# jasperzhong/GNNFlow

Measured on AMD Instinct MI355X. Metric: sampled_edges_per_s, higher is better.
Workload: dtype int64/f32

## Files before the change

gnnflow_amd/csrc/sample_layer.hip:

```cpp
#include "sampler_ctx.hpp"

#include <cstdlib>

#include "../../include/gnnflow_rng.h"

namespace gf {

namespace {

__global__ void sample_publish_kernel(Publish p) {
  if (threadIdx.x != 0 || blockIdx.x != 0) return;
  for (uint32_t i = 0; i < p.num_words; ++i) p.h_counts[i] = p.d_counts[i];
  p.h_counts[p.num_words] = p.d_extra ? *p.d_extra : 0;
  __threadfence_system();
  *reinterpret_cast<volatile uint64_t*>(p.h_flag) = p.seq;
}

__global__ void sample_publish_group_kernel(PublishGroup g) {
  if (threadIdx.x != 0) return;
  const Publish& p = g.p[blockIdx.x];
  for (uint32_t i = 0; i < p.num_words; ++i) p.h_counts[i] = p.d_counts[i];
  p.h_counts[p.num_words] = p.d_extra ? *p.d_extra : 0;
  __threadfence_system();
  *reinterpret_cast<volatile uint64_t*>(p.h_flag) = p.seq;
}

template <int GROUP>
__global__ __launch_bounds__(kSearchThreads) void sample_search_kernel(
    GraphView g, const int64_t* __restrict__ roots, const float* __restrict__ root_ts,
    const uint64_t* __restrict__ d_R, uint64_t R_host, uint32_t snapshot_idx,
    uint32_t num_snapshots, float window, uint64_t* __restrict__ rec_end,
    uint32_t* __restrict__ rec_cnt, uint32_t fanout, int uniform,
    uint32_t* __restrict__ wg_sum, const uint32_t* __restrict__ list,
    const uint32_t* __restrict__ seg_count, uint32_t num_segs, uint32_t seg_cap) {
  __shared__ uint32_t s_sum;
  __shared__ uint32_t seg_prefix[kMaxHubSegs + 1];
  if (wg_sum && threadIdx.x == 0) s_sum = 0;
  if (wg_sum) __syncthreads();
  uint64_t R = d_R ? *d_R : R_host;
  if (list) {
    __shared__ uint32_t wtot[kSearchThreads / 64];
    uint32_t carry = 0;
    for (uint32_t s0 = 0; s0 < num_segs; s0 += kSearchThreads) {
      const uint32_t sidx = s0 + threadIdx.x;
      const uint32_t v = sidx < num_segs ? seg_count[sidx] : 0u;
      uint32_t incl = v;
#pragma unroll
      for (int d = 1; d < 64; d <<= 1) {
        const uint32_t up = __shfl_up(incl, d, 64);
        if ((threadIdx.x & 63) >= d) incl += up;
      }
      __syncthreads();
      if ((threadIdx.x & 63) == 63) wtot[threadIdx.x >> 6] = incl;
      __syncthreads();
      uint32_t wbase = 0, tot = 0;
      for (int w = 0; w < kSearchThreads / 64; ++w) {
        if (w < (threadIdx.x >> 6)) wbase += wtot[w];
        tot += wtot[w];
      }
      if (sidx < num_segs) seg_prefix[sidx] = carry + wbase + incl - v;
      carry += tot;
    }
    if (threadIdx.x == 0) seg_prefix[num_segs] = carry;
    __syncthreads();
    R = seg_prefix[num_segs];
  }
  constexpr int kGroupsPerBlock = kSearchThreads / GROUP;
  const int lane = threadIdx.x % GROUP;
  const int group_in_wave = (threadIdx.x % 64) / GROUP;
  const uint64_t group = static_cast<uint64_t>(blockIdx.x) * kGroupsPerBlock + threadIdx.x / GROUP;
  const uint64_t num_groups = static_cast<uint64_t>(gridDim.x) * kGroupsPerBlock;
  for (uint64_t i = group; i < R; i += num_groups) {
    uint64_t r = i;
    if (list) {
      uint32_t lo_s = 0, hi_s = num_segs;
      while (hi_s - lo_s > 1) {
        const uint32_t mid = (lo_s + hi_s) >> 1;
        if (seg_prefix[mid] <= i) lo_s = mid; else hi_s = mid;
      }
      r = list[static_cast<uint64_t>(lo_s) * seg_cap + (i - seg_prefix[lo_s])];
    }
    const int64_t nid = roots[r];
    const float t = root_ts[r];
    float start, end;
    time_window(t, snapshot_idx, num_snapshots, window, &start, &end);
    uint64_t end_off = 0;
    uint32_t n_cand = 0;
    if (nid >= 0 && static_cast<uint64_t>(nid) < g.table_len) {
      const NodeEntry e = g.table[nid];
      if (e.size > 0) {
        uint32_t lo, hi;
        window_bounds<GROUP>(g, e, start, end, lane, group_in_wave, &lo, &hi);
        n_cand = hi > lo ? hi - lo : 0;
        end_off = e.start + hi;
      }
    }
    if (lane == 0) {
      rec_end[r] = end_off;
      rec_cnt[r] = n_cand;
      if (wg_sum) atomicAdd(&s_sum, valid_slots(n_cand, fanout, uniform));
    }
  }
  if (wg_sum) {
    __syncthreads();
    if (threadIdx.x == 0) wg_sum[blockIdx.x] = s_sum;
  }
}

constexpr uint32_t kLaneDeg = 16;

__global__ __launch_bounds__(kSearchThreads) void sample_search_lanes_kernel(
    GraphView g, const int64_t* __restrict__ roots, const float* __restrict__ root_ts,
    const uint64_t* __restrict__ d_R, uint64_t R_host, uint32_t snapshot_idx,
    uint32_t num_snapshots, float window, uint64_t* __restrict__ rec_end,
    uint32_t* __restrict__ rec_cnt, uint32_t* __restrict__ hub_list,
    uint32_t* __restrict__ seg_count, uint32_t seg_cap) {
  __shared__ uint32_t s_seg_n;
  if (threadIdx.x == 0) s_seg_n = 0;
  __syncthreads();
  uint32_t* seg = hub_list + static_cast<uint64_t>(blockIdx.x) * seg_cap;
  const uint64_t R = d_R ? *d_R : R_host;
  const int lane = threadIdx.x & 63;
  const uint64_t wave = (static_cast<uint64_t>(blockIdx.x) * kSearchThreads + threadIdx.x) >> 6;
  const uint64_t num_waves = (static_cast<uint64_t>(gridDim.x) * kSearchThreads) >> 6;
  const uint64_t chunks = (R + 63) / 64;
  for (uint64_t chunk = wave; chunk < chunks; chunk += num_waves) {
    const uint64_t r = chunk * 64 + lane;
    const bool in = r < R;
    int64_t nid = -1;
    float start = 0.f, end = 0.f;
    if (in) {
      nid = roots[r];
      time_window(root_ts[r], snapshot_idx, num_snapshots, window, &start, &end);
    }
    NodeEntry e;
    e.start = 0;
    e.size = 0;
    if (in && nid >= 0 && static_cast<uint64_t>(nid) < g.table_len) e = g.table[nid];
    const bool whole = g.nonneg_ts > 0 && start <= 0.0f && e.size > 0 &&
                       end > __uint_as_float(e.last_ts_bits);
    const bool big = e.size > kLaneDeg && !whole;
    if (in && whole) {
      rec_end[r] = e.start + e.size;
      rec_cnt[r] = e.size;
    } else if (in && !big) {
      uint32_t hi = 0, lo = 0;
      if (e.size > 0) {
        const float* ts = g.ts_pool + e.start;
        float v[kLaneDeg];
        if ((e.start & 3u) == 0) {
          const float4* t4 = reinterpret_cast<const float4*>(ts);
#pragma unroll
          for (uint32_t q = 0; q < kLaneDeg / 4; ++q) {
            const float4 x = 4 * q < e.size ? t4[q] : make_float4(0.f, 0.f, 0.f, 0.f);
            v[4 * q] = x.x; v[4 * q + 1] = x.y; v[4 * q + 2] = x.z; v[4 * q + 3] = x.w;
          }
        } else {
#pragma unroll
          for (uint32_t i = 0; i < kLaneDeg; ++i) v[i] = i < e.size ? ts[i] : 0.f;
// ... 181 lines not shown
    pub.h_counts[pub.num_words] = 0;
  }
  const uint64_t stride = static_cast<uint64_t>(gridDim.x) * blockDim.x;
  const uint64_t first = static_cast<uint64_t>(blockIdx.x) * blockDim.x + threadIdx.x;
  constexpr int K = 4;
  for (uint64_t t0 = first; t0 < total; t0 += K * stride) {
    uint64_t t[K], r[K], end[K];
    uint32_t j[K], n[K], bs[K];
    float rts[K];
    bool in[K];
#pragma unroll
    for (int k = 0; k < K; ++k) {
      t[k] = t0 + static_cast<uint64_t>(k) * stride;
      in[k] = t[k] < total;
      r[k] = in[k] ? t[k] / fanout : 0;
      j[k] = static_cast<uint32_t>(t[k] - r[k] * fanout);
    }
#pragma unroll
    for (int k = 0; k < K; ++k) {
      n[k] = in[k] ? rec_cnt[r[k]] : 0u;
      end[k] = in[k] ? rec_end[r[k]] : 0;
      bs[k] = in[k] ? base[r[k]] : 0u;
      rts[k] = in[k] ? root_ts[r[k]] : 0.f;
      if (in[k] && t[k] < R) {
        all_nodes[t[k]] = roots[t[k]];
        all_ts[t[k]] = root_ts[t[k]];
      }
    }
    EdgePair nb[K];
    bool ok[K];
#pragma unroll
    for (int k = 0; k < K; ++k) {
      ok[k] = in[k] && j[k] < valid_slots(n[k], fanout, uniform);
      if (ok[k]) {
        const uint32_t pick = uniform ? gf_philox4x32_10_first(seed, t[k], call) % n[k] : j[k];
        nb[k] = g.nbr_pool[end[k] - 1 - pick];
      }
    }
#pragma unroll
    for (int k = 0; k < K; ++k) {
      if (!ok[k]) continue;
      const float ets = nb[k].ts;
      const uint64_t o = static_cast<uint64_t>(bs[k]) + j[k];
      all_nodes[R + o] = nb[k].dst;
      all_ts[R + o] = prop_time ? rts[k] : ets;
      dt[o] = rts[k] - ets;
      eids[o] = nb[k].eid;
      row[o] = static_cast<int64_t>(r[k]);
      col[o] = static_cast<int64_t>(R + o);
    }
  }
}

__global__ __launch_bounds__(kEmitThreads) void sample_emit_prefix_kernel(
    GraphView g, const int64_t* __restrict__ roots, const float* __restrict__ root_ts,
    const uint64_t* d_R, uint64_t R_host, uint32_t fanout, int uniform, int prop_time,
    uint64_t seed, uint64_t call, const uint64_t* __restrict__ rec_end,
    const uint32_t* __restrict__ rec_cnt, const uint32_t* __restrict__ wg_sum,
    uint32_t roots_per_search_wg, int64_t* __restrict__ all_nodes, float* __restrict__ all_ts,
    float* __restrict__ dt, int64_t* __restrict__ eids, int64_t* __restrict__ row,
    int64_t* __restrict__ col, uint64_t* out_R, uint64_t* out_S, uint64_t* next_R, Publish pub) {
  __shared__ uint32_t red[kEmitThreads / 64];
  __shared__ uint32_t lbase[kEmitThreads];
  __shared__ uint32_t wave_tot[kEmitThreads / 64];
  const uint64_t R = d_R ? *d_R : R_host;
  const uint64_t total = R * fanout;
  const uint64_t t0 = static_cast<uint64_t>(blockIdx.x) * kEmitThreads;
  if (t0 >= total) return;
  const int tid = threadIdx.x, lane = tid & 63, wave = tid >> 6;
  const uint64_t t_last = min(t0 + kEmitThreads - 1, total - 1);
  const uint32_t r_first = static_cast<uint32_t>(t0 / fanout);
  const uint32_t r_last = static_cast<uint32_t>(t_last / fanout);
  const uint32_t nroots = r_last - r_first + 1;
  const uint32_t b_first = r_first / roots_per_search_wg;
  uint32_t part = 0;
  for (uint32_t b = tid; b < b_first; b += kEmitThreads) part += wg_sum[b];
  for (uint32_t r = b_first * roots_per_search_wg + tid; r < r_first; r += kEmitThreads)
    part += valid_slots(rec_cnt[r], fanout, uniform);
  for (int d = 32; d > 0; d >>= 1) part += __shfl_down(part, d, 64);
  if (lane == 0) red[wave] = part;
  const uint32_t mine = tid < static_cast<int>(nroots)
                            ? valid_slots(rec_cnt[r_first + tid], fanout, uniform) : 0u;
  uint32_t incl = mine;
#pragma unroll
  for (int d = 1; d < 64; d <<= 1) {
    uint32_t up = __shfl_up(incl, d, 64);
    if (lane >= d) incl += up;
  }
  if (lane == 63) wave_tot[wave] = incl;
  __syncthreads();
  uint32_t base = 0;
#pragma unroll
  for (int w = 0; w < kEmitThreads / 64; ++w) base += red[w];
  uint32_t wbase = 0;
  for (int w = 0; w < wave; ++w) wbase += wave_tot[w];
  lbase[tid] = base + wbase + incl - mine;
  __syncthreads();
  const uint64_t t = t0 + tid;
  if (t < total) {
    if (t < R) {
      all_nodes[t] = roots[t];
      all_ts[t] = root_ts[t];
    }
    const uint32_t r = static_cast<uint32_t>(t / fanout);
    const uint32_t j = static_cast<uint32_t>(t - static_cast<uint64_t>(r) * fanout);
    const uint32_t n = rec_cnt[r];
    if (j < valid_slots(n, fanout, uniform)) {
      const uint32_t pick = uniform ? gf_philox4x32_10_first(seed, t, call) % n : j;
      const uint64_t e = rec_end[r] - 1 - pick;
      const EdgePair nb = g.nbr_pool[e];
      const float ets = nb.ts;
      const float rts = root_ts[r];
      const uint64_t o = static_cast<uint64_t>(lbase[r - r_first]) + j;
      all_nodes[R + o] = nb.dst;
      all_ts[R + o] = prop_time ? rts : ets;
      dt[o] = rts - ets;
      eids[o] = nb.eid;
      row[o] = static_cast<int64_t>(r);
      col[o] = static_cast<int64_t>(R + o);
    }
  }
  if (t_last == total - 1 && tid == static_cast<int>(nroots) - 1) {
    const uint64_t S = static_cast<uint64_t>(lbase[tid]) + mine;
    *out_R = R;
    *out_S = S;
    if (next_R) *next_R = R + S;
    for (uint32_t i = 0; i < pub.num_words; ++i) pub.h_counts[i] = pub.d_counts[i];
    if (pub.num_words) pub.h_counts[pub.num_words] = 0;
  }
}

template <typename... Args>
void launch_search(int width, unsigned grid, hipStream_t stream, Args... args) {
  switch (width) {
    case 2: sample_search_kernel<2><<<dim3(grid), dim3(kSearchThreads), 0, stream>>>(args...); break;
    case 4: sample_search_kernel<4><<<dim3(grid), dim3(kSearchThreads), 0, stream>>>(args...); break;
    case 8: sample_search_kernel<8><<<dim3(grid), dim3(kSearchThreads), 0, stream>>>(args...); break;
    default: sample_search_kernel<16><<<dim3(grid), dim3(kSearchThreads), 0, stream>>>(args...); break;
  }
}

}

int group_width_from_env(const char* name, int fallback) {
  const char* v = std::getenv(name);
  const int g = v ? std::atoi(v) : fallback;
  return (g == 2 || g == 4 || g == 8 || g == 16) ? g : fallback;
}

void launch_scan(const uint32_t* rec_cnt, uint32_t* base, uint32_t* tile_scratch,
                 const uint64_t* d_R, uint64_t R_host, size_t Rb, uint32_t F, int uniform,
                 uint64_t* out_R, uint64_t* out_S, uint64_t* next_R, hipStream_t stream) {
  if (Rb <= 65536) {
    sample_scan_kernel<<<dim3(1), dim3(kScanThreads), 0, stream>>>(
        rec_cnt, base, d_R, R_host, F, uniform, out_R, out_S, next_R);
    return;
  }
  const size_t tiles = (Rb + kScanTile - 1) / kScanTile;
  uint32_t* tile_sum = tile_scratch;
  uint32_t* tile_base = tile_scratch + tiles;
  const unsigned grid = static_cast<unsigned>(std::min<size_t>(tiles, 2048));
  sample_tile_sum_kernel<<<dim3(grid), dim3(kScanThreads), 0, stream>>>(
      rec_cnt, d_R, R_host, F, uniform, tile_sum);
  sample_tile_scan_kernel<<<dim3(1), dim3(kScanThreads), 0, stream>>>(
      tile_sum, tile_base, d_R, R_host, out_R, out_S, next_R);
  sample_tile_apply_kernel<<<dim3(grid), dim3(kScanThreads), 0, stream>>>(
      rec_cnt, tile_base, d_R, R_host, F, uniform, base);
}

void launch_publish(const Publish& p, hipStream_t stream) {
  sample_publish_kernel<<<dim3(1), dim3(64), 0, stream>>>(p);
}
void launch_publish_group(const PublishGroup& g, int m, hipStream_t stream) {
  sample_publish_group_kernel<<<dim3(static_cast<unsigned>(m)), dim3(64), 0, stream>>>(g);
}

void Sampler::enqueue_layer(const int64_t* d_roots, const float* d_ts, size_t Rb,
                            const uint64_t* d_R, uint64_t R_host, uint32_t layer,
                            uint32_t snapshot, const BlockPtrs& out, uint64_t* d_counts_slot,
                            uint64_t* next_R, hipStream_t stream, const Publish& pub) {
  const uint32_t F = fanouts_[layer];
  const int uniform = policy_ == GF_SAMPLING_POLICY_UNIFORM;
  GF_REQUIRE(static_cast<uint64_t>(Rb) * F < 0xFFFFFFFFull,
             "sampler: more than 2^32-1 slots in one layer");
  char* w = ws_.as<char>();
  uint64_t* rec_end = reinterpret_cast<uint64_t*>(w); w += align_up(ws_roots_ * 8, 16);
  uint32_t* rec_cnt = reinterpret_cast<uint32_t*>(w); w += align_up(ws_roots_ * 4, 16);
  uint32_t* base = reinterpret_cast<uint32_t*>(w);    w += align_up(ws_roots_ * 4, 16);
  uint32_t* wg_sum = reinterpret_cast<uint32_t*>(w);
  const GraphView gv = view_for(graph_, Rb);
  const uint64_t call = calls_++;
  const bool small = Rb <= kSmallRoots;
  const unsigned roots_per_wg = kSearchThreads / search_group_;
  {
    ProfileScope ps(kProfSearch, stream);
    const unsigned grid = small ? static_cast<unsigned>((Rb + roots_per_wg - 1) / roots_per_wg)
                                : capped_grid(Rb, roots_per_wg, 256 * 8);
    if (hybrid_search_ && Rb >= kLaneSearchRoots) {
      const unsigned lgrid = capped_grid(Rb, kSearchThreads, kMaxHubSegs);
      const uint64_t chunks_per_wg = ((Rb + 63) / 64 + (lgrid * 4ull) - 1) / (lgrid * 4ull);
      const uint32_t seg_cap = static_cast<uint32_t>(chunks_per_wg * 4 * 64);
      const size_t hub_bytes = static_cast<size_t>(seg_cap) * lgrid * sizeof(uint32_t);
      if (hub_bytes > hub_buf_.bytes()) {
        DeviceBuffer fresh;
        fresh.reserve(hub_bytes, 0, stream);
        std::swap(hub_buf_, fresh);
        retired_.retire(std::move(fresh), stream);
      }
      uint32_t* hub_list_ = hub_buf_.as<uint32_t>();
      uint32_t* seg_count = wg_sum;
      sample_search_lanes_kernel<<<dim3(lgrid), dim3(kSearchThreads), 0, stream>>>(
          gv, d_roots, d_ts, d_R, R_host, snapshot, num_snapshots_, window_, rec_end, rec_cnt,
          hub_list_, seg_count, seg_cap);
      launch_search(large_group_, capped_grid(Rb / 4, kSearchThreads / large_group_, 256 * 8),
                    stream, gv, d_roots, d_ts, nullptr, 0, snapshot, num_snapshots_, window_,
                    rec_end, rec_cnt, F, uniform, nullptr, hub_list_, seg_count, lgrid, seg_cap);
    } else if (small) {
      launch_search(search_group_, grid, stream, gv, d_roots, d_ts, d_R, R_host, snapshot,
                    num_snapshots_, window_, rec_end, rec_cnt, F, uniform, wg_sum, nullptr,
                    nullptr, 0, 0);
    } else {
      launch_search(large_group_, capped_grid(Rb, kSearchThreads / large_group_, 256 * 8), stream,
                    gv, d_roots, d_ts, d_R, R_host, snapshot, num_snapshots_, window_, rec_end,
                    rec_cnt, F, uniform, nullptr, nullptr, nullptr, 0, 0);
    }
    GF_HIP(hipGetLastError());
  }
  if (small) {
    ProfileScope ps(kProfEmit, stream);
    const unsigned grid = static_cast<unsigned>(
        (static_cast<uint64_t>(Rb) * F + kEmitThreads - 1) / kEmitThreads);
    sample_emit_prefix_kernel<<<dim3(grid), dim3(kEmitThreads), 0, stream>>>(
        gv, d_roots, d_ts, d_R, R_host, F, uniform, prop_time_ ? 1 : 0, seed_, call, rec_end,
        rec_cnt, wg_sum, roots_per_wg, out.all_nodes, out.all_ts, out.dt, out.eids, out.row,
        out.col, d_counts_slot, d_counts_slot + 1, next_R, pub);
    GF_HIP(hipGetLastError());
    return;
  }
  {
    ProfileScope ps(kProfScan, stream);
    launch_scan(rec_cnt, base, wg_sum, d_R, R_host, Rb, F, uniform, d_counts_slot,
                d_counts_slot + 1, next_R, stream);
    GF_HIP(hipGetLastError());
  }
  {
    ProfileScope ps(kProfEmit, stream);
    unsigned grid = capped_grid(static_cast<uint64_t>(Rb) * F, kEmitThreads, 256 * 16);
    sample_emit_kernel<<<dim3(grid), dim3(kEmitThreads), 0, stream>>>(
        gv, d_roots, d_ts, d_R, R_host, F, uniform, prop_time_ ? 1 : 0, seed_, call, rec_end,
        rec_cnt, base, out.all_nodes, out.all_ts, out.dt, out.eids, out.row, out.col, pub);
    GF_HIP(hipGetLastError());
  }
}

__global__ void philox_debug_kernel(const uint64_t* __restrict__ in, size_t n,
                                    uint32_t* __restrict__ out) {
  const size_t i = static_cast<size_t>(blockIdx.x) * blockDim.x + threadIdx.x;
  if (i < n) out[i] = gf_philox4x32_10_first(in[3 * i], in[3 * i + 1], in[3 * i + 2]);
}
void philox_on_device(const uint64_t* d_in, size_t n, uint32_t* d_out, hipStream_t stream) {
  if (n == 0) return;
  philox_debug_kernel<<<dim3(static_cast<unsigned>((n + 255) / 256)), dim3(256), 0, stream>>>(
      d_in, n, d_out);
  GF_HIP(hipGetLastError());
}

}
```

gnnflow_amd/csrc/sampler.hip:

```cpp
#include "sampler_ctx.hpp"
#include "partition.hpp"

#include <sched.h>

#include <atomic>
#include <chrono>
#include <cmath>
#include <cstdlib>
#include <cstring>

namespace gf {

Sampler::Sampler(EdgeStore* graph, const uint32_t* fanouts, size_t num_layers, int policy,
                 uint32_t num_snapshots, float window, bool prop_time, uint64_t seed)
    : graph_(graph),
      fanouts_(fanouts, fanouts + num_layers),
      policy_(policy),
      num_snapshots_(num_snapshots),
      window_(window),
      prop_time_(prop_time),
      seed_(seed) {
  GF_REQUIRE(graph != nullptr, "sampler: null graph");
  GF_REQUIRE(num_layers > 0, "sampler: fanouts must not be empty");
  for (uint32_t f : fanouts_) GF_REQUIRE(f > 0, "sampler: fanout must be positive");
// ... 13 lines not shown
  std::memset(h_counts_.data(), 0, kMaxInFlight * rec_words_ * sizeof(uint64_t));
  h_layer_counts_.reserve(2 * sizeof(uint64_t));
}

Sampler::~Sampler() {
  for (InFlight& f : ring_) {
    if (f.done) {
      (void)hipEventSynchronize(f.done);
      (void)hipEventDestroy(f.done);
    }
  }
  if (own_stream_) {
    (void)hipStreamSynchronize(own_stream_);
    (void)hipStreamDestroy(own_stream_);
  }
}

size_t Sampler::root_bound(size_t R, size_t layer) const {
  size_t b = R;
  for (size_t l = 0; l < layer; ++l) b += b * fanouts_[l];
  return b;
}

size_t Sampler::layer_output_bytes(size_t Rb, size_t layer) const {
  const size_t F = fanouts_[layer], Sb = Rb * F;
  return align_up((Rb + Sb) * 8, 16) + align_up((Rb + Sb) * 4, 16) + align_up(Sb * 4, 16) +
         3 * align_up(Sb * 8, 16);
}

Sampler::BlockPtrs Sampler::carve(char* p, size_t Rb, uint32_t F) const {
  const size_t Sb = Rb * F;
  BlockPtrs b;
  b.all_nodes = reinterpret_cast<int64_t*>(p); p += align_up((Rb + Sb) * 8, 16);
  b.eids = reinterpret_cast<int64_t*>(p);      p += align_up(Sb * 8, 16);
  b.row = reinterpret_cast<int64_t*>(p);       p += align_up(Sb * 8, 16);
  b.col = reinterpret_cast<int64_t*>(p);       p += align_up(Sb * 8, 16);
  b.all_ts = reinterpret_cast<float*>(p);      p += align_up((Rb + Sb) * 4, 16);
  b.dt = reinterpret_cast<float*>(p);
  return b;
}

size_t Sampler::output_bytes(size_t R) const {
  size_t total = 0;
  for (size_t l = 0; l < fanouts_.size(); ++l)
    total += num_snapshots_ * layer_output_bytes(root_bound(R, l), l);
  return total;
}

void Sampler::reserve_workspace(size_t Rb, size_t num_blocks, hipStream_t stream) {
  if (Rb <= ws_roots_ && num_blocks <= ws_blocks_) return;
  ws_roots_ = std::max(ws_roots_, Rb);
  ws_blocks_ = std::max(ws_blocks_, num_blocks);
  size_t bytes = align_up(ws_roots_ * 8, 16) + 3 * align_up(ws_roots_ * 4, 16) +
                 ws_blocks_ * 2 * sizeof(uint64_t) + 64;
  retired_.collect();
  DeviceBuffer fresh;
  fresh.reserve(bytes, 0, stream);
  GF_HIP(hipMemsetAsync(fresh.data(), 0, align_up(ws_roots_ * 8, 16), stream));
  std::swap(ws_, fresh);
  retired_.retire(std::move(fresh), stream);
}

void Sampler::sample_begin(const int64_t* d_roots, const float* d_ts, size_t R, void* d_out,
                           size_t out_bytes, hipStream_t stream) {
  const size_t L = fanouts_.size(), NS = num_snapshots_;
  InFlight* slot;
  {
    std::lock_guard<std::mutex> lk(ring_mu_);
    GF_REQUIRE(ring_count_ < kMaxInFlight, "sample_begin: too many samples in flight on this sampler");
    if (ring_count_ > 0) {
      const InFlight& newest = ring_[(ring_head_ + ring_count_ - 1) % kMaxInFlight];
      GF_REQUIRE(newest.roots == 0 || R == 0 || newest.stream == stream,
                 "sample_begin: samples in flight on one sampler must share a stream");
    }
    slot = &ring_[(ring_head_ + ring_count_) % kMaxInFlight];
  }
  slot->ptrs.assign(L * NS, BlockPtrs{});
  slot->roots = R;
  slot->by_event = false;
  slot->stream = stream;
  if (R == 0) {
    calls_ += L * NS;
    std::lock_guard<std::mutex> lk(ring_mu_);
    ++ring_count_;
    return;
  }
  GF_REQUIRE(d_roots && d_ts && d_out, "sample: null device pointer");
  GF_REQUIRE(out_bytes >= output_bytes(R), "sample: output buffer too small");
  DeviceGuard dg(graph_->device());
  reserve_workspace(root_bound(R, L - 1), L * NS, stream);
  uint64_t* d_counts = reinterpret_cast<uint64_t*>(
      ws_.as<char>() + align_up(ws_roots_ * 8, 16) + 3 * align_up(ws_roots_ * 4, 16));

  std::vector<BlockPtrs>& ptrs = slot->ptrs;
  char* p = static_cast<char*>(d_out);
  for (size_t l = 0; l < L; ++l) {
    const size_t Rb = root_bound(R, l);
    for (size_t s = 0; s < NS; ++s) {
      ptrs[l * NS + s] = carve(p, Rb, fanouts_[l]);
      p += layer_output_bytes(Rb, l);
    }
  }
  slot->seq = ++publish_seq_;
  uint64_t* rec = h_counts_.as<uint64_t>() + (slot->seq % kMaxInFlight) * rec_words_;
  *reinterpret_cast<volatile uint64_t*>(rec) = 0;
  Publish pub;
  pub.d_counts = d_counts;
  pub.h_counts = rec + 1;
  pub.h_flag = rec;
  pub.seq = slot->seq;
  pub.num_words = static_cast<uint32_t>(L * NS * 2);
  slot->by_event = true;
  for (size_t l = 0; l < L; ++l) {
    const size_t Rb = root_bound(R, l);
    for (size_t s = 0; s < NS; ++s) {
      const size_t b = l * NS + s;
      uint64_t* cslot = d_counts + 2 * b;
      uint64_t* next_R = (l + 1 < L) ? cslot + 2 * NS : nullptr;
      const Publish last = (b + 1 == L * NS) ? pub : Publish{};
      if (l == 0) {
        enqueue_layer(d_roots, d_ts, Rb, nullptr, R, l, s, ptrs[b], cslot, next_R, stream, last);
      } else {
        const BlockPtrs& prev = ptrs[(l - 1) * NS + s];
        enqueue_layer(prev.all_nodes, prev.all_ts, Rb, cslot, 0, l, s, ptrs[b], cslot, next_R,
                      stream, last);
      }
    }
  }
  GF_HIP(hipEventRecord(slot->done, stream));
  std::lock_guard<std::mutex> lk(ring_mu_);
  ++ring_count_;
}

size_t Sampler::in_flight() const {
  std::lock_guard<std::mutex> lk(ring_mu_);
  return ring_count_;
}

void Sampler::sample_end(gf_block* blocks) {
  const size_t L = fanouts_.size(), NS = num_snapshots_;
  GF_REQUIRE(blocks != nullptr, "sample: null blocks array");
  InFlight* slot;
  {
    std::lock_guard<std::mutex> lk(ring_mu_);
    GF_REQUIRE(ring_count_ > 0, "sample_end: no sample in flight");
    slot = &ring_[ring_head_];
  }
  auto pop = [&] {
    std::lock_guard<std::mutex> lk(ring_mu_);
    ring_head_ = (ring_head_ + 1) % kMaxInFlight;
    --ring_count_;
  };
  if (slot->roots == 0) {
    for (size_t b = 0; b < L * NS; ++b) std::memset(&blocks[b], 0, sizeof(gf_block));
    last_overflow_ = false;
    pop();
    return;
  }
  DeviceGuard dg(graph_->device());
  const uint64_t* rec = h_counts_.as<uint64_t>() + (slot->seq % kMaxInFlight) * rec_words_;
  volatile const uint64_t* flag = rec;
  bool seen = false;
  if (slot->by_event) {
    for (uint64_t spin = 0;; ++spin) {
      const hipError_t q = hipEventQuery(slot->done);
      if (q == hipSuccess) break;
      if (q != hipErrorNotReady) { pop(); GF_HIP(q); }
      if (spin > 4096 && (spin & 63) == 0) sched_yield();
    }
    seen = true;
  }
  for (uint64_t spin = 0; !seen && spin < (1ull << 26); ++spin) {
    if (*flag == slot->seq) { seen = true; break; }
    __builtin_ia32_pause();
    if (spin > 4096 && (spin & 63) == 0) sched_yield();
  }
  if (!seen) {
    const hipError_t e = hipEventSynchronize(slot->done);
    if (e != hipSuccess) { pop(); GF_HIP(e); }
  }
  __atomic_thread_fence(__ATOMIC_ACQUIRE);
  const uint64_t* hc = rec + 1;
  for (size_t b = 0; b < L * NS; ++b) {
    gf_block& o = blocks[b];
    o.all_nodes = slot->ptrs[b].all_nodes;
    o.all_timestamps = slot->ptrs[b].all_ts;
    o.delta_timestamps = slot->ptrs[b].dt;
    o.eids = slot->ptrs[b].eids;
    o.row = slot->ptrs[b].row;
    o.col = slot->ptrs[b].col;
    o.num_dst_nodes = hc[2 * b];
    o.num_edges = hc[2 * b + 1];
    o.num_src_nodes = o.num_dst_nodes + o.num_edges;
  }
  last_overflow_ = hc[2 * L * NS] != 0;
  pop();
}

void Sampler::sample(const int64_t* d_roots, const float* d_ts, size_t R, void* d_out,
                     size_t out_bytes, gf_block* blocks, hipStream_t stream) {
  GF_REQUIRE(blocks != nullptr, "sample: null blocks array");
  sample_begin(d_roots, d_ts, R, d_out, out_bytes, stream);
  sample_end(blocks);
}

void Sampler::sample_layer(const int64_t* d_roots, const float* d_ts, size_t R, uint32_t layer,
                           uint32_t snapshot, void* d_out, size_t out_bytes, gf_block* block,
                           hipStream_t stream) {
  GF_REQUIRE(layer < fanouts_.size(), "sample_layer: layer out of range");
  GF_REQUIRE(snapshot < num_snapshots_, "sample_layer: snapshot out of range");
  GF_REQUIRE(block != nullptr, "sample_layer: null block");
  if (R == 0) {
    std::memset(block, 0, sizeof(gf_block));
    calls_++;
    return;
  }
  GF_REQUIRE(d_roots && d_ts && d_out, "sample_layer: null device pointer");
  GF_REQUIRE(out_bytes >= layer_output_bytes(R, layer), "sample_layer: output buffer too small");
  DeviceGuard dg(graph_->device());
  reserve_workspace(R, 2, stream);
  uint64_t* d_counts = reinterpret_cast<uint64_t*>(
      ws_.as<char>() + align_up(ws_roots_ * 8, 16) + 3 * align_up(ws_roots_ * 4, 16));
  BlockPtrs ptrs = carve(static_cast<char*>(d_out), R, fanouts_[layer]);
  enqueue_layer(d_roots, d_ts, R, nullptr, R, layer, snapshot, ptrs, d_counts, nullptr, stream,
                Publish{});
  GF_HIP(hipMemcpyAsync(h_layer_counts_.data(), d_counts, 2 * sizeof(uint64_t),
                        hipMemcpyDeviceToHost, stream));
  GF_HIP(hipStreamSynchronize(stream));
  const uint64_t* hc = h_layer_counts_.as<uint64_t>();
  block->all_nodes = ptrs.all_nodes;
  block->all_timestamps = ptrs.all_ts;
  block->delta_timestamps = ptrs.dt;
  block->eids = ptrs.eids;
  block->row = ptrs.row;
  block->col = ptrs.col;
  block->num_dst_nodes = hc[0];
  block->num_edges = hc[1];
  block->num_src_nodes = hc[0] + hc[1];
}

std::atomic<uint64_t> g_part_host_ns[8];
void part_host_add(int stage, uint64_t v) {
  g_part_host_ns[stage].fetch_add(v, std::memory_order_relaxed);
}

void Sampler::part_layout(size_t R0, uint32_t layer, int world_size, double slack,
                          size_t slot_roots, gf_part_layout* out, bool skip_prev) const {
  GF_REQUIRE(layer < fanouts_.size(), "part_layout: layer out of range");
  GF_REQUIRE(out != nullptr, "part_layout: null output");
  GF_REQUIRE(slack >= 0.0, "part_layout: negative slack");
  const size_t Rb = root_bound(R0, layer), F = fanouts_[layer];
  size_t stride = 0, rows = Rb;
  if (slack > 0.0) {
    const size_t Sb = root_bound(std::max<size_t>(slot_roots, 1), layer) -
                      ((skip_prev && layer > 0) ? root_bound(std::max<size_t>(slot_roots, 1), layer - 1) : 0);
    const double share = std::ceil(static_cast<double>(Sb) * slack / world_size);
    const size_t cap = std::max<size_t>(1, std::min<size_t>(Sb, static_cast<size_t>(share)));
    stride = cap + 1;
    rows = static_cast<size_t>(world_size) * stride + Rb;
    GF_REQUIRE(rows < 0xFFFFFFFFull, "part_layout: more than 2^32-1 request rows");
  }
  out->root_bound = Rb;
  out->requests = 0;
  out->replies = rows * 16;
  out->counts = out->replies + rows * F * 24;
  out->pos = out->counts + align_up(static_cast<size_t>(world_size) * 8, 16);
  out->scratch = align_up(out->pos + Rb * 4, 16);
  out->scratch_bytes = partition_scratch_bytes(Rb, world_size);
  size_t end = align_up(out->scratch + out->scratch_bytes, 256);
  out->slot_stride = stride;
  out->inbox = out->served = 0;
  if (stride) {
    const size_t slots = static_cast<size_t>(world_size) * stride;
    out->inbox = end;
    out->served = align_up(out->inbox + slots * 16, 256);
    end = align_up(out->served + slots * F * 24, 256);
  }
  out->total = end;
// ... 305 lines not shown
```

gnnflow_amd/csrc/sampler.hpp:

```cpp
#pragma once

#include <cstdint>
#include <mutex>
#include <vector>

#include "comm.hpp"
#include "common.hpp"
#include "edge_store.hpp"

namespace gf {

struct Publish;

class Sampler {
 public:
  Sampler(EdgeStore* graph, const uint32_t* fanouts, size_t num_layers, int policy,
          uint32_t num_snapshots, float window, bool prop_time, uint64_t seed);
  ~Sampler();

  size_t num_layers() const { return fanouts_.size(); }
  uint32_t fanout(size_t layer) const { return fanouts_[layer]; }
  uint32_t num_snapshots() const { return num_snapshots_; }
  int device() const { return graph_->device(); }

// ... 24 lines not shown
  void part_serve(uint32_t layer, uint32_t snapshot, void* d_ws, size_t ws_bytes,
                  bool with_own = false);
  bool last_overflow() const { return last_overflow_; }
  void part_plan_own(uint32_t layer, uint32_t snapshot, void* d_ws, size_t ws_bytes, int phases);
  void part_merge(uint32_t layer, uint32_t snapshot, void* d_ws, size_t ws_bytes);
  void part_commit();
  void part_abort();
  static constexpr int kMaxGroup = 4;
  struct GroupSample {
    Sampler* s;
    const int64_t* d_roots;
    const float* d_ts;
    size_t R;
    void* d_out;
    size_t out_bytes;
  };
  struct GroupLayout {
    size_t stride, slot_rows, own[kMaxGroup];
    size_t requests, replies, inbox, served, counts[kMaxGroup], pos[kMaxGroup], total;
    size_t first[kMaxGroup];
    size_t edge_cap, off_bytes, cslot, row_cnt, cserved, creplies;
  };
  bool group_ok(const size_t* R, int m) const;
  bool layer_reuses_roots(bool reuse_roots, size_t layer) const {
    return reuse_roots && layer > 0 && policy_ != GF_SAMPLING_POLICY_UNIFORM &&
           fanouts_[layer] == fanouts_[layer - 1];
  }
  void group_layout(const size_t* R, int m, uint32_t layer, int world, double slack,
                    size_t slot_roots, bool narrow, double edge_fill, GroupLayout* out,
                    bool reuse_roots = false) const;
  static size_t group_ws_bytes(const Sampler& a, const size_t* R, int m, int world, double slack,
                               size_t slot_roots, bool narrow, double edge_fill = 0.0,
                               bool reuse_roots = false);
  static void sample_partitioned_group(const GroupSample* gs, int m, void* d_ws, size_t ws_bytes,
                                       double slack, size_t slot_roots, Exchange* ex,
                                       hipStream_t stream, unsigned force_overflow = 0,
                                       bool narrow = false, double edge_fill = 0.0,
                                       bool reuse_roots = false);
  void sample_partitioned(const int64_t* d_roots, const float* d_ts, size_t R, void* d_out,
                          size_t out_bytes, void* d_ws, size_t ws_bytes, hipStream_t stream);
  void sample_partitioned_slotted(const int64_t* d_roots, const float* d_ts, size_t R, void* d_out,
                                  size_t out_bytes, void* d_ws, size_t ws_bytes, double slack,
                                  size_t slot_roots, Exchange& ex, bool overlap,
                                  hipStream_t stream);
  void sample_host(const int64_t* nodes, const float* ts, size_t R, gf_block* blocks);
  void sample_layer_host(const int64_t* nodes, const float* ts, size_t R, uint32_t layer,
                         uint32_t snapshot, gf_block* block);

 private:
  struct BlockPtrs {
    int64_t* all_nodes; float* all_ts; float* dt; int64_t* eids; int64_t* row; int64_t* col;
  };
  BlockPtrs carve(char* base, size_t Rb, uint32_t fanout) const;
  void enqueue_layer(const int64_t* d_roots, const float* d_ts, size_t R_bound,
                     const uint64_t* d_R, uint64_t R_host, uint32_t layer, uint32_t snapshot,
                     const BlockPtrs& out, uint64_t* d_counts_slot, uint64_t* next_R,
                     hipStream_t stream, const Publish& publish);
  void reserve_workspace(size_t R_bound_max, size_t num_blocks, hipStream_t stream);
  void to_host_blocks(const gf_block* dev, gf_block* host, size_t n, hipStream_t stream);

  EdgeStore* graph_;
  std::vector<uint32_t> fanouts_;
  int policy_;
  uint32_t num_snapshots_;
  float window_;
  bool prop_time_;
  uint64_t seed_;
  DeviceBuffer part_ticket_;
  uint32_t part_tag_ = 0;
  uint64_t calls_ = 0;
 public:
  uint64_t call_counter() const { return calls_; }
  void set_call_counter(uint64_t v) { calls_ = v; }
 private:
  int search_group_ = 16;
  int large_group_ = 4;
  bool hybrid_search_ = true;
  struct InFlight {
    size_t roots = 0;
    uint64_t seq = 0;
    hipStream_t stream = nullptr;
    hipEvent_t done = nullptr;
    bool by_event = false;
    std::vector<BlockPtrs> ptrs;
  };
  struct PartState {
    bool active = false;
    InFlight* slot = nullptr;
    const int64_t* d_roots = nullptr;
    const float* d_ts = nullptr;
    size_t R = 0, Rs = 1;
    int world = 1, rank = 0;
    double slack = 0.0;
    size_t slot_roots = 0;
    hipStream_t stream = nullptr;
  };
  uint64_t* part_counts() const;
  uint32_t* part_overflow() const;
  bool last_overflow_ = false;
  uint32_t* part_rec_cnt() const;
  uint32_t* part_root_of() const;
  bool part_own_counts(size_t root_bound) const;
  bool part_fused_merge(size_t root_bound, uint32_t fanout) const;
  void part_commit_prepare(Publish& pub);
  void part_commit_finish();
  void part_roots(uint32_t layer, uint32_t snapshot, const int64_t** roots, const float** ts,
                  const uint64_t** d_R, uint64_t* R_host) const;
  InFlight ring_[kMaxInFlight];
  size_t ring_head_ = 0, ring_count_ = 0;
  mutable std::mutex ring_mu_;
// ... 20 lines not shown
```

gnnflow_amd/csrc/sampler_ctx.hpp:

```cpp
#pragma once

#include "sampler.hpp"

#include <algorithm>

namespace gf {

constexpr int kSearchThreads = 256;
constexpr int kEmitThreads = 256;
constexpr int kScanThreads = 1024;
constexpr int kScanItems = 4;
constexpr size_t kSmallRoots = 32768;
constexpr uint32_t kGranuleSpins = 1u << 12;
constexpr size_t kLaneSearchRoots = size_t{1} << 20;
constexpr uint32_t kMaxHubSegs = 2048;
constexpr int kScanTile = 4096;
constexpr int kCompactThreads = 1024;
constexpr uint64_t kGranuleCountMask = 0x3FF;

__device__ inline void time_window(float root_ts, uint32_t snapshot_idx,
                                   uint32_t num_snapshots, float window, float* start,
                                   float* end) {
  if (num_snapshots == 1) {
    *start = (fabs(static_cast<double>(window)) < 1e-6) ? 0.0f : root_ts - window;
    *end = root_ts;
  } else {
    float k = static_cast<float>(num_snapshots - snapshot_idx - 1);
    *end = fmaf(-k, window, root_ts);
    *start = *end - window;
  }
}

template <int GROUP>
__device__ inline uint32_t group_count(bool pred, int group_in_wave) {
  unsigned long long m = __ballot(pred);
  if (GROUP == 64) return __popcll(m);
  return __popcll((m >> (group_in_wave * GROUP)) & ((1ull << GROUP) - 1ull));
}

template <int GROUP>
__device__ inline uint32_t lower_bound_group(const float* __restrict__ ts, uint32_t n,
                                             float x, int lane, int group_in_wave) {
  uint32_t lo = 0, hi = n;
  while (hi - lo > GROUP) {
    uint32_t span = hi - lo;
    uint32_t stride = (span + GROUP - 1) / GROUP;
    uint32_t p = lo + lane * stride;
    bool less = (p < hi) && (ts[p] < x);
    uint32_t c = group_count<GROUP>(less, group_in_wave);
    if (c == 0) {
      hi = lo;
    } else {
      uint32_t nlo = lo + (c - 1) * stride + 1;
      uint32_t nhi = lo + c * stride;
      hi = nhi < hi ? nhi : hi;
      lo = nlo;
    }
  }
  uint32_t p = lo + lane;
  bool less = (p < hi) && (ts[p] < x);
  return lo + group_count<GROUP>(less, group_in_wave);
}

template <int GROUP>
__device__ inline uint32_t lower_bound_fenced(const GraphView& g, uint64_t s, uint32_t n, float x,
// ... 239 lines not shown
```

Before: 762.2 million.

## Fuse next-layer neighbor search into emit kernel for small multi-layer batches

For small batches with a single snapshot, the emit kernel of layer l now also runs the time-window search for the newly produced roots of layer l+1. It writes rec_end/rec_cnt and accumulates per-workgroup slot sums into rotating fused sum buffers, so the separate search launch for the next layer is skipped. A head search kernel also zeroes the sum buffers, replacing separate memsets. This removes kernel launches and a pass over the new roots, at the cost of small 32-slot emit tiles with low occupancy per block and atomics on global sums.

```diff
diff --git a/gnnflow_amd/csrc/sample_layer.hip b/gnnflow_amd/csrc/sample_layer.hip
--- a/gnnflow_amd/csrc/sample_layer.hip
+++ b/gnnflow_amd/csrc/sample_layer.hip
@@ -23,6 +23,26 @@
   p.h_counts[p.num_words] = p.d_extra ? *p.d_extra : 0;
   __threadfence_system();
   *reinterpret_cast<volatile uint64_t*>(p.h_flag) = p.seq;
+}
+
+template <int GROUP>
+__device__ __forceinline__ void search_root(const GraphView& g, int64_t nid, float t,
+                                            uint32_t snapshot_idx, uint32_t num_snapshots,
+                                            float window, int lane, int group_in_wave,
+                                            uint64_t* end_off, uint32_t* n_cand) {
+  float start, end;
+  time_window(t, snapshot_idx, num_snapshots, window, &start, &end);
+  *end_off = 0;
+  *n_cand = 0;
+  if (nid >= 0 && static_cast<uint64_t>(nid) < g.table_len) {
+    const NodeEntry e = g.table[nid];
+    if (e.size > 0) {
+      uint32_t lo, hi;
+      window_bounds<GROUP>(g, e, start, end, lane, group_in_wave, &lo, &hi);
+      *n_cand = hi > lo ? hi - lo : 0;
+      *end_off = e.start + hi;
+    }
+  }
 }
 
 template <int GROUP>
@@ -80,21 +100,10 @@
       }
       r = list[static_cast<uint64_t>(lo_s) * seg_cap + (i - seg_prefix[lo_s])];
     }
-    const int64_t nid = roots[r];
-    const float t = root_ts[r];
-    float start, end;
-    time_window(t, snapshot_idx, num_snapshots, window, &start, &end);
-    uint64_t end_off = 0;
-    uint32_t n_cand = 0;
-    if (nid >= 0 && static_cast<uint64_t>(nid) < g.table_len) {
-      const NodeEntry e = g.table[nid];
-      if (e.size > 0) {
-        uint32_t lo, hi;
-        window_bounds<GROUP>(g, e, start, end, lane, group_in_wave, &lo, &hi);
-        n_cand = hi > lo ? hi - lo : 0;
-        end_off = e.start + hi;
-      }
-    }
+    uint64_t end_off;
+    uint32_t n_cand;
+    search_root<GROUP>(g, roots[r], root_ts[r], snapshot_idx, num_snapshots, window, lane,
+                       group_in_wave, &end_off, &n_cand);
     if (lane == 0) {
       rec_end[r] = end_off;
       rec_cnt[r] = n_cand;
@@ -105,6 +114,37 @@
     __syncthreads();
     if (threadIdx.x == 0) wg_sum[blockIdx.x] = s_sum;
   }
+}
+
+template <int GROUP>
+__global__ __launch_bounds__(kSearchThreads) void sample_search_head_kernel(
+    GraphView g, const int64_t* __restrict__ roots, const float* __restrict__ root_ts,
+    uint64_t R, uint32_t snapshot_idx, uint32_t num_snapshots, float window,
+    uint64_t* __restrict__ rec_end, uint32_t* __restrict__ rec_cnt, uint32_t fanout, int uniform,
+    uint32_t* __restrict__ wg_sum, uint32_t* __restrict__ zero, uint32_t zero_n) {
+  __shared__ uint32_t s_sum;
+  if (threadIdx.x == 0) s_sum = 0;
+  for (uint32_t i = blockIdx.x * kSearchThreads + threadIdx.x; i < zero_n;
+       i += gridDim.x * kSearchThreads)
+    zero[i] = 0;
+  __syncthreads();
+  constexpr int kGroupsPerBlock = kSearchThreads / GROUP;
+  const int lane = threadIdx.x % GROUP;
+  const int group_in_wave = (threadIdx.x % 64) / GROUP;
+  const uint64_t r = static_cast<uint64_t>(blockIdx.x) * kGroupsPerBlock + threadIdx.x / GROUP;
+  if (r < R) {
+    uint64_t end_off;
+    uint32_t n_cand;
+    search_root<GROUP>(g, roots[r], root_ts[r], snapshot_idx, num_snapshots, window, lane,
+                       group_in_wave, &end_off, &n_cand);
+    if (lane == 0) {
+      rec_end[r] = end_off;
+      rec_cnt[r] = n_cand;
+      atomicAdd(&s_sum, valid_slots(n_cand, fanout, uniform));
+    }
+  }
+  __syncthreads();
+  if (threadIdx.x == 0) wg_sum[blockIdx.x] = s_sum;
 }
 
 constexpr uint32_t kLaneDeg = 16;
@@ -392,23 +432,53 @@
   }
 }
 
-__global__ __launch_bounds__(kEmitThreads) void sample_emit_prefix_kernel(
-    GraphView g, const int64_t* __restrict__ roots, const float* __restrict__ root_ts,
-    const uint64_t* d_R, uint64_t R_host, uint32_t fanout, int uniform, int prop_time,
-    uint64_t seed, uint64_t call, const uint64_t* __restrict__ rec_end,
-    const uint32_t* __restrict__ rec_cnt, const uint32_t* __restrict__ wg_sum,
-    uint32_t roots_per_search_wg, int64_t* __restrict__ all_nodes, float* __restrict__ all_ts,
-    float* __restrict__ dt, int64_t* __restrict__ eids, int64_t* __restrict__ row,
-    int64_t* __restrict__ col, uint64_t* out_R, uint64_t* out_S, uint64_t* next_R, Publish pub) {
+struct EmitArgs {
+  GraphView g;
+  const int64_t* roots;
+  const float* root_ts;
+  const uint64_t* d_R;
+  uint64_t R_host;
+  uint32_t fanout;
+  int uniform, prop_time;
+  uint64_t seed, call;
+  const uint64_t* rec_end;
+  const uint32_t* rec_cnt;
+  const uint32_t* wg_sum;
+  uint32_t roots_per_search_wg;
+  int64_t* all_nodes; float* all_ts; float* dt; int64_t* eids; int64_t* row; int64_t* col;
+  uint64_t* out_R; uint64_t* out_S; uint64_t* next_R;
+  Publish pub;
+};
+
+struct NewRoot {
+  bool valid;
+  uint32_t o;
+  int64_t node;
+  float ts;
+};
+
+template <int TILE>
+__device__ __forceinline__ bool emit_prefix_tile(const EmitArgs& a, uint64_t* R_out, NewRoot* nr,
+                                                 uint32_t* o_first) {
+  static_assert(TILE >= 16 && TILE <= kEmitThreads, "a tile is at most one slot per thread");
   __shared__ uint32_t red[kEmitThreads / 64];
-  __shared__ uint32_t lbase[kEmitThreads];
+  __shared__ uint32_t lbase[TILE];
   __shared__ uint32_t wave_tot[kEmitThreads / 64];
-  const uint64_t R = d_R ? *d_R : R_host;
+  const int64_t* __restrict__ roots = a.roots;
+  const float* __restrict__ root_ts = a.root_ts;
+  const uint64_t* __restrict__ rec_end = a.rec_end;
+  const uint32_t* __restrict__ rec_cnt = a.rec_cnt;
+  const uint32_t* __restrict__ wg_sum = a.wg_sum;
+  const uint32_t fanout = a.fanout, roots_per_search_wg = a.roots_per_search_wg;
+  const int uniform = a.uniform;
+  const uint64_t R = a.d_R ? *a.d_R : a.R_host;
+  *R_out = R;
+  nr->valid = false;
   const uint64_t total = R * fanout;
-  const uint64_t t0 = static_cast<uint64_t>(blockIdx.x) * kEmitThreads;
-  if (t0 >= total) return;
+  const uint64_t t0 = static_cast<uint64_t>(blockIdx.x) * TILE;
+  if (t0 >= total) return false;
   const int tid = threadIdx.x, lane = tid & 63, wave = tid >> 6;
-  const uint64_t t_last = min(t0 + kEmitThreads - 1, total - 1);
+  const uint64_t t_last = min(t0 + TILE - 1, total - 1);
   const uint32_t r_first = static_cast<uint32_t>(t0 / fanout);
   const uint32_t r_last = static_cast<uint32_t>(t_last / fanout);
   const uint32_t nroots = r_last - r_first + 1;
@@ -434,40 +504,119 @@
   for (int w = 0; w < kEmitThreads / 64; ++w) base += red[w];
   uint32_t wbase = 0;
   for (int w = 0; w < wave; ++w) wbase += wave_tot[w];
-  lbase[tid] = base + wbase + incl - mine;
-  __syncthreads();
+  if (tid < TILE) lbase[tid] = base + wbase + incl - mine;
+  __syncthreads();
+  {
+    const uint32_t j0 = static_cast<uint32_t>(t0 - static_cast<uint64_t>(r_first) * fanout);
+    const uint32_t v0 = valid_slots(rec_cnt[r_first], fanout, uniform);
+    *o_first = lbase[0] + (j0 < v0 ? j0 : v0);
+  }
   const uint64_t t = t0 + tid;
-  if (t < total) {
+  if (tid < TILE && t < total) {
     if (t < R) {
-      all_nodes[t] = roots[t];
-      all_ts[t] = root_ts[t];
+      a.all_nodes[t] = roots[t];
+      a.all_ts[t] = root_ts[t];
     }
     const uint32_t r = static_cast<uint32_t>(t / fanout);
     const uint32_t j = static_cast<uint32_t>(t - static_cast<uint64_t>(r) * fanout);
     const uint32_t n = rec_cnt[r];
     if (j < valid_slots(n, fanout, uniform)) {
-      const uint32_t pick = uniform ? gf_philox4x32_10_first(seed, t, call) % n : j;
+      const uint32_t pick = uniform ? gf_philox4x32_10_first(a.seed, t, a.call) % n : j;
       const uint64_t e = rec_end[r] - 1 - pick;
-      const EdgePair nb = g.nbr_pool[e];
+      const EdgePair nb = a.g.nbr_pool[e];
       const float ets = nb.ts;
       const float rts = root_ts[r];
       const uint64_t o = static_cast<uint64_t>(lbase[r - r_first]) + j;
-      all_nodes[R + o] = nb.dst;
-      all_ts[R + o] = prop_time ? rts : ets;
-      dt[o] = rts - ets;
-      eids[o] = nb.eid;
-      row[o] = static_cast<int64_t>(r);
-      col[o] = static_cast<int64_t>(R + o);
+      a.all_nodes[R + o] = nb.dst;
+      a.all_ts[R + o] = a.prop_time ? rts : ets;
+      a.dt[o] = rts - ets;
+      a.eids[o] = nb.eid;
+      a.row[o] = static_cast<int64_t>(r);
+      a.col[o] = static_cast<int64_t>(R + o);
+      nr->valid = true;
+      nr->o = static_cast<uint32_t>(o);
+      nr->node = nb.dst;
+      nr->ts = a.prop_time ? rts : ets;
     }
   }
   if (t_last == total - 1 && tid == static_cast<int>(nroots) - 1) {
     const uint64_t S = static_cast<uint64_t>(lbase[tid]) + mine;
-    *out_R = R;
-    *out_S = S;
-    if (next_R) *next_R = R + S;
-    for (uint32_t i = 0; i < pub.num_words; ++i) pub.h_counts[i] = pub.d_counts[i];
-    if (pub.num_words) pub.h_counts[pub.num_words] = 0;
-  }
+    *a.out_R = R;
+    *a.out_S = S;
+    if (a.next_R) *a.next_R = R + S;
+    for (uint32_t i = 0; i < a.pub.num_words; ++i) a.pub.h_counts[i] = a.pub.d_counts[i];
+    if (a.pub.num_words) a.pub.h_counts[a.pub.num_words] = 0;
+  }
+  return true;
+}
+
+__global__ __launch_bounds__(kEmitThreads) void sample_emit_prefix_kernel(EmitArgs a) {
+  uint64_t R;
+  NewRoot nr;
+  uint32_t o_first;
+  emit_prefix_tile<kEmitThreads>(a, &R, &nr, &o_first);
+}
+
+struct NextSearchArgs {
+  uint32_t snapshot_idx, num_snapshots;
+  float window;
+  uint32_t fanout;
+  uint64_t* rec_end;
+  uint32_t* rec_cnt;
+  uint32_t* sum_next;
+  uint32_t* zero;
+  uint32_t zero_n;
+};
+
+template <int TILE, int GROUP>
+__global__ __launch_bounds__(kEmitThreads) void sample_emit_search_kernel(EmitArgs a,
+                                                                          NextSearchArgs s) {
+  constexpr int kAcc = TILE / 16 + 2;
+  __shared__ int64_t s_node[TILE];
+  __shared__ float s_ts[TILE];
+  __shared__ uint32_t s_acc[kAcc];
+  __shared__ uint32_t s_n;
+  const int tid = threadIdx.x;
+  for (uint32_t i = blockIdx.x * kEmitThreads + tid; i < s.zero_n; i += gridDim.x * kEmitThreads)
+    s.zero[i] = 0;
+  if (tid < kAcc) s_acc[tid] = 0;
+  if (tid == 0) s_n = 0;
+  uint64_t R;
+  NewRoot nr;
+  uint32_t o_first;
+  if (!emit_prefix_tile<TILE>(a, &R, &nr, &o_first)) return;
+  const uint32_t rpw = a.roots_per_search_wg;
+  const uint64_t t = static_cast<uint64_t>(blockIdx.x) * TILE + tid;
+  if (tid < TILE && t < R)
+    atomicAdd(&s.sum_next[t / rpw], valid_slots(a.rec_cnt[t], s.fanout, a.uniform));
+  if (nr.valid) {
+    const uint32_t p = nr.o - o_first;
+    if (p < TILE) {
+      s_node[p] = nr.node;
+      s_ts[p] = nr.ts;
+      atomicMax(&s_n, p + 1);
+    }
+  }
+  __syncthreads();
+  constexpr int kGroups = kEmitThreads / GROUP;
+  const int lane = tid % GROUP, group_in_wave = (tid % 64) / GROUP;
+  const uint32_t n_new = s_n;
+  const uint64_t first = R + o_first;
+  const uint64_t w0 = first / rpw;
+  for (uint32_t i = tid / GROUP; i < n_new; i += kGroups) {
+    uint64_t end_off;
+    uint32_t n_cand;
+    search_root<GROUP>(a.g, s_node[i], s_ts[i], s.snapshot_idx, s.num_snapshots, s.window, lane,
+                       group_in_wave, &end_off, &n_cand);
+    if (lane == 0) {
+      s.rec_end[first + i] = end_off;
+      s.rec_cnt[first + i] = n_cand;
+      const uint64_t w = (first + i) / rpw - w0;
+      if (w < kAcc) atomicAdd(&s_acc[w], valid_slots(n_cand, s.fanout, a.uniform));
+    }
+  }
+  __syncthreads();
+  if (tid < kAcc && s_acc[tid]) atomicAdd(&s.sum_next[w0 + tid], s_acc[tid]);
 }
 
 template <typename... Args>
@@ -477,6 +626,16 @@
     case 4: sample_search_kernel<4><<<dim3(grid), dim3(kSearchThreads), 0, stream>>>(args...); break;
     case 8: sample_search_kernel<8><<<dim3(grid), dim3(kSearchThreads), 0, stream>>>(args...); break;
     default: sample_search_kernel<16><<<dim3(grid), dim3(kSearchThreads), 0, stream>>>(args...); break;
+  }
+}
+
+template <typename... Args>
+void launch_search_head(int width, unsigned grid, hipStream_t stream, Args... args) {
+  switch (width) {
+    case 2: sample_search_head_kernel<2><<<dim3(grid), dim3(kSearchThreads), 0, stream>>>(args...); break;
+    case 4: sample_search_head_kernel<4><<<dim3(grid), dim3(kSearchThreads), 0, stream>>>(args...); break;
+    case 8: sample_search_head_kernel<8><<<dim3(grid), dim3(kSearchThreads), 0, stream>>>(args...); break;
+    default: sample_search_head_kernel<16><<<dim3(grid), dim3(kSearchThreads), 0, stream>>>(args...); break;
   }
 }
 
@@ -518,7 +677,8 @@
 void Sampler::enqueue_layer(const int64_t* d_roots, const float* d_ts, size_t Rb,
                             const uint64_t* d_R, uint64_t R_host, uint32_t layer,
                             uint32_t snapshot, const BlockPtrs& out, uint64_t* d_counts_slot,
-                            uint64_t* next_R, hipStream_t stream, const Publish& pub) {
+                            uint64_t* next_R, hipStream_t stream, const Publish& pub,
+                            LayerFusion fuse) {
   const uint32_t F = fanouts_[layer];
   const int uniform = policy_ == GF_SAMPLING_POLICY_UNIFORM;
   GF_REQUIRE(static_cast<uint64_t>(Rb) * F < 0xFFFFFFFFull,
@@ -531,8 +691,19 @@
   const GraphView gv = view_for(graph_, Rb);
   const uint64_t call = calls_++;
   const bool small = Rb <= kSmallRoots;
+  const bool chained = fuse.searched || fuse.search_next;
   const unsigned roots_per_wg = kSearchThreads / search_group_;
-  {
+  if (chained) wg_sum = fused_sums(layer % 3);
+  if (fuse.searched) {
+  } else if (fuse.search_next) {
+    ProfileScope ps(kProfSearch, stream);
+    const unsigned grid = static_cast<unsigned>((Rb + roots_per_wg - 1) / roots_per_wg);
+    const size_t next_words = (Rb * (1 + static_cast<size_t>(F))) / roots_per_wg + 1;
+    launch_search_head(search_group_, grid, stream, gv, d_roots, d_ts, R_host, snapshot,
+                       num_snapshots_, window_, rec_end, rec_cnt, F, uniform, wg_sum,
+                       fused_sums((layer + 1) % 3), static_cast<uint32_t>(next_words));
+    GF_HIP(hipGetLastError());
+  } else {
     ProfileScope ps(kProfSearch, stream);
     const unsigned grid = small ? static_cast<unsigned>((Rb + roots_per_wg - 1) / roots_per_wg)
                                 : capped_grid(Rb, roots_per_wg, 256 * 8);
@@ -568,12 +739,35 @@
   }
   if (small) {
     ProfileScope ps(kProfEmit, stream);
-    const unsigned grid = static_cast<unsigned>(
-        (static_cast<uint64_t>(Rb) * F + kEmitThreads - 1) / kEmitThreads);
-    sample_emit_prefix_kernel<<<dim3(grid), dim3(kEmitThreads), 0, stream>>>(
-        gv, d_roots, d_ts, d_R, R_host, F, uniform, prop_time_ ? 1 : 0, seed_, call, rec_end,
-        rec_cnt, wg_sum, roots_per_wg, out.all_nodes, out.all_ts, out.dt, out.eids, out.row,
-        out.col, d_counts_slot, d_counts_slot + 1, next_R, pub);
+    EmitArgs a;
+    a.g = gv;
+    a.roots = d_roots; a.root_ts = d_ts; a.d_R = d_R; a.R_host = R_host;
+    a.fanout = F; a.uniform = uniform; a.prop_time = prop_time_ ? 1 : 0;
+    a.seed = seed_; a.call = call;
+    a.rec_end = rec_end; a.rec_cnt = rec_cnt; a.wg_sum = wg_sum;
+    a.roots_per_search_wg = roots_per_wg;
+    a.all_nodes = out.all_nodes; a.all_ts = out.all_ts; a.dt = out.dt; a.eids = out.eids;
+    a.row = out.row; a.col = out.col;
+    a.out_R = d_counts_slot; a.out_S = d_counts_slot + 1; a.next_R = next_R;
+    a.pub = pub;
+    const uint64_t slots = static_cast<uint64_t>(Rb) * F;
+    if (fuse.search_next) {
+      const uint32_t F1 = fanouts_[layer + 1];
+      NextSearchArgs s;
+      s.snapshot_idx = snapshot; s.num_snapshots = num_snapshots_; s.window = window_;
+      s.fanout = F1;
+      s.rec_end = rec_end; s.rec_cnt = rec_cnt;
+      s.sum_next = fused_sums((layer + 1) % 3);
+      s.zero = fused_sums((layer + 2) % 3);
+      const size_t Rb2 = (Rb + slots) * (1 + static_cast<size_t>(F1));
+      s.zero_n = fuse.zero_after_next ? static_cast<uint32_t>(Rb2 / roots_per_wg + 1) : 0u;
+      const unsigned grid = static_cast<unsigned>((slots + kFusedTile - 1) / kFusedTile);
+      sample_emit_search_kernel<kFusedTile, kFusedGroup>
+          <<<dim3(grid), dim3(kEmitThreads), 0, stream>>>(a, s);
+    } else {
+      const unsigned grid = static_cast<unsigned>((slots + kEmitThreads - 1) / kEmitThreads);
+      sample_emit_prefix_kernel<<<dim3(grid), dim3(kEmitThreads), 0, stream>>>(a);
+    }
     GF_HIP(hipGetLastError());
     return;
   }
diff --git a/gnnflow_amd/csrc/sampler.hip b/gnnflow_amd/csrc/sampler.hip
--- a/gnnflow_amd/csrc/sampler.hip
+++ b/gnnflow_amd/csrc/sampler.hip
@@ -89,13 +89,20 @@
   ws_roots_ = std::max(ws_roots_, Rb);
   ws_blocks_ = std::max(ws_blocks_, num_blocks);
   size_t bytes = align_up(ws_roots_ * 8, 16) + 3 * align_up(ws_roots_ * 4, 16) +
-                 ws_blocks_ * 2 * sizeof(uint64_t) + 64;
+                 ws_blocks_ * 2 * sizeof(uint64_t) + 64 +
+                 3 * align_up(fused_sum_words() * 4, 16);
   retired_.collect();
   DeviceBuffer fresh;
   fresh.reserve(bytes, 0, stream);
   GF_HIP(hipMemsetAsync(fresh.data(), 0, align_up(ws_roots_ * 8, 16), stream));
   std::swap(ws_, fresh);
   retired_.retire(std::move(fresh), stream);
+}
+
+uint32_t* Sampler::fused_sums(uint32_t k) const {
+  return reinterpret_cast<uint32_t*>(
+      ws_.as<char>() + align_up(ws_roots_ * 8, 16) + 3 * align_up(ws_roots_ * 4, 16) +
+      ws_blocks_ * 2 * sizeof(uint64_t) + 64 + k * align_up(fused_sum_words() * 4, 16));
 }
 
 void Sampler::sample_begin(const int64_t* d_roots, const float* d_ts, size_t R, void* d_out,
@@ -155,12 +162,18 @@
       uint64_t* cslot = d_counts + 2 * b;
       uint64_t* next_R = (l + 1 < L) ? cslot + 2 * NS : nullptr;
       const Publish last = (b + 1 == L * NS) ? pub : Publish{};
+      auto fuses = [&](size_t k) { return NS == 1 && k + 1 < L && root_bound(R, k + 1) <= kSmallRoots; };
+      LayerFusion fuse;
+      fuse.searched = l > 0 && fuses(l - 1);
+      fuse.search_next = fuses(l);
+      fuse.zero_after_next = fuses(l + 1);
       if (l == 0) {
-        enqueue_layer(d_roots, d_ts, Rb, nullptr, R, l, s, ptrs[b], cslot, next_R, stream, last);
+        enqueue_layer(d_roots, d_ts, Rb, nullptr, R, l, s, ptrs[b], cslot, next_R, stream, last,
+                      fuse);
       } else {
         const BlockPtrs& prev = ptrs[(l - 1) * NS + s];
         enqueue_layer(prev.all_nodes, prev.all_ts, Rb, cslot, 0, l, s, ptrs[b], cslot, next_R,
-                      stream, last);
+                      stream, last, fuse);
       }
     }
   }
@@ -260,7 +273,7 @@
       ws_.as<char>() + align_up(ws_roots_ * 8, 16) + 3 * align_up(ws_roots_ * 4, 16));
   BlockPtrs ptrs = carve(static_cast<char*>(d_out), R, fanouts_[layer]);
   enqueue_layer(d_roots, d_ts, R, nullptr, R, layer, snapshot, ptrs, d_counts, nullptr, stream,
-                Publish{});
+                Publish{}, LayerFusion{});
   GF_HIP(hipMemcpyAsync(h_layer_counts_.data(), d_counts, 2 * sizeof(uint64_t),
                         hipMemcpyDeviceToHost, stream));
   GF_HIP(hipStreamSynchronize(stream));
diff --git a/gnnflow_amd/csrc/sampler.hpp b/gnnflow_amd/csrc/sampler.hpp
--- a/gnnflow_amd/csrc/sampler.hpp
+++ b/gnnflow_amd/csrc/sampler.hpp
@@ -100,10 +100,15 @@
     int64_t* all_nodes; float* all_ts; float* dt; int64_t* eids; int64_t* row; int64_t* col;
   };
   BlockPtrs carve(char* base, size_t Rb, uint32_t fanout) const;
+  struct LayerFusion {
+    bool searched = false, search_next = false, zero_after_next = false;
+  };
   void enqueue_layer(const int64_t* d_roots, const float* d_ts, size_t R_bound,
                      const uint64_t* d_R, uint64_t R_host, uint32_t layer, uint32_t snapshot,
                      const BlockPtrs& out, uint64_t* d_counts_slot, uint64_t* next_R,
-                     hipStream_t stream, const Publish& publish);
+                     hipStream_t stream, const Publish& publish, LayerFusion fuse);
+  size_t fused_sum_words() const { return ws_roots_ / 16 + 1; }
+  uint32_t* fused_sums(uint32_t k) const;
   void reserve_workspace(size_t R_bound_max, size_t num_blocks, hipStream_t stream);
   void to_host_blocks(const gf_block* dev, gf_block* host, size_t n, hipStream_t stream);
 
diff --git a/gnnflow_amd/csrc/sampler_ctx.hpp b/gnnflow_amd/csrc/sampler_ctx.hpp
--- a/gnnflow_amd/csrc/sampler_ctx.hpp
+++ b/gnnflow_amd/csrc/sampler_ctx.hpp
@@ -11,6 +11,8 @@
 constexpr int kScanThreads = 1024;
 constexpr int kScanItems = 4;
 constexpr size_t kSmallRoots = 32768;
+constexpr int kFusedTile = 32;
+constexpr int kFusedGroup = 8;
 constexpr uint32_t kGranuleSpins = 1u << 12;
 constexpr size_t kLaneSearchRoots = size_t{1} << 20;
 constexpr uint32_t kMaxHubSegs = 2048;
```

New measurement: 738.9 million. -3.1%, worse.
